# rubychen0611/image-analogies-python

Measured on AMD Instinct MI355X. Metric: B' pixels/sec (brute-force match, 5-level pyramid) + MFMA util @1/2/4/8 GPU, higher is better.
Workload: dtype f16 rotated split (R16 MFMA screen: 3 principal components as f16 pairs, 52 as f16, f32 accumulate) + f64 (rotation, exact rescore, pyramids); 1 GPU; c4: A/A' 2048x2048 x B 1024x1024, 5-level, DB sharded, brute force; levels_cap=5, jobs_per_gpu=1, streams_per_gpu=1, jobs_per_launch=1, parallelism=single

## Files before the change

### image-analogies-python_amd/csrc/ia_screen16r.hip

```cpp
#include "ia_internal.h"
#include "ia_rot16.h"
#include "../../include/ia_diag.h"

#include <float.h>
#include <type_traits>

namespace ia {
namespace {

typedef float floatx16 __attribute__((ext_vector_type(16)));
constexpr int STAGE_TILES = 4;
constexpr int STAGE_H8 = STAGE_TILES * R16_TILE_H8;
constexpr int MAX_G = 11;
constexpr int SPC_MAX = 16;
#ifndef IA_R16_RING
#define IA_R16_RING 2
#endif
#ifndef IA_R16_OCC
#define IA_R16_OCC 4
#endif
constexpr int R16_RING = IA_R16_RING;
#ifndef IA_R16_NTMIN
#define IA_R16_NTMIN 0
#endif
#ifndef IA_R16_PIN
#define IA_R16_PIN 1
#endif
#ifndef IA_R16_SPC
#define IA_R16_SPC 2
#endif
constexpr int SPC_STAGE = IA_R16_SPC;
#ifndef IA_RK_TILES
#define IA_RK_TILES 4
#endif
#ifndef IA_RK_RING
#define IA_RK_RING 2
#endif
#ifndef IA_RK_SPC
#define IA_RK_SPC 8
#endif
#ifndef IA_RK_OCC
#define IA_RK_OCC 4
#endif
constexpr int RK_TILES = IA_RK_TILES, RK_RING = IA_RK_RING, RK_SPC = IA_RK_SPC;
static_assert(RK_TILES == 4 || RK_TILES == 8, "a compact stage is one or two 128-row stages of the stage map");
static_assert(RK_RING >= 2 && R16_RING >= 2 && RK_SPC >= 1 && RK_SPC <= 16, "stage ring, staged minima");

__host__ __device__ constexpr int bal_t0(int G, int W) { return (G * W) / 4; }
__host__ __device__ constexpr int bal_ns(int G, int W) { return (G * W + G - 1) / 4 - (G * W) / 4 + 1; }
__host__ __device__ constexpr bool bal_on(int G, int W, int k, int u) {
    return 4 * (bal_t0(G, W) + k) + u >= G * W && 4 * (bal_t0(G, W) + k) + u < G * W + G;
}
template <int G, int W>
__host__ __device__ constexpr int ch_count() {
    int n = 0;
    for (int u = 0; u < STAGE_TILES; ++u)
        for (int k = 0; k < bal_ns(G, W); ++k) n += bal_on(G, W, k, u) ? 1 : 0;
    return n;
}
template <int G, int W>
__host__ __device__ constexpr int ch_u(int c) {
    for (int u = 0; u < STAGE_TILES; ++u)
        for (int k = 0; k < bal_ns(G, W); ++k)
            if (bal_on(G, W, k, u) && c-- == 0) return u;
    return -1;
}
template <int G, int W>
__host__ __device__ constexpr int ch_k(int c) {
    for (int u = 0; u < STAGE_TILES; ++u)
        for (int k = 0; k < bal_ns(G, W); ++k)
            if (bal_on(G, W, k, u) && c-- == 0) return k;
    return -1;
}
template <int G, int W>
__host__ __device__ constexpr int ch_uo(int c) {
    int o = 0;
    for (int i = 1; i <= c; ++i) o += ch_u<G, W>(i) != ch_u<G, W>(i - 1) ? 1 : 0;
    return o;
}
template <int G, int W>
__host__ __device__ constexpr int ch_next(int c) {
    for (int i = c + 1; i < ch_count<G, W>(); ++i)
        if (ch_u<G, W>(i) != ch_u<G, W>(c)) return i;
    return -1;
}
template <int G, int W>
__host__ __device__ constexpr bool ch_first(int c) { return c == 0 || ch_u<G, W>(c) != ch_u<G, W>(c - 1); }
#ifndef IA_R16_PF
#define IA_R16_PF 1
#endif
template <int G, int W>
__host__ __device__ constexpr bool ch_reads_next(int c) {
    return IA_R16_PF ? (ch_first<G, W>(c) && ch_next<G, W>(c) >= 0)
                     : (c + 1 < ch_count<G, W>() && ch_u<G, W>(c + 1) != ch_u<G, W>(c));
}
template <int K, int N, typename F>
__device__ __forceinline__ void sfor(F &&f) {
    if constexpr (K < N) {
        f(std::integral_constant<int, K>{});
        sfor<K + 1, N>(f);
    }
}
__device__ __forceinline__ int fkey(float x) {
    const int b = __float_as_int(x);
    return b >= 0 ? b : b ^ 0x7fffffff;
}
__device__ __forceinline__ float fkey_inv(int b) { return __int_as_float(b >= 0 ? b : b ^ 0x7fffffff); }
__device__ __forceinline__ void fold_min(const floatx16 &x, float &mn) {
    const float t0 = fminf(fminf(x[0], x[1]), x[2]), t1 = fminf(fminf(x[3], x[4]), x[5]);
    const float t2 = fminf(fminf(x[6], x[7]), x[8]), t3 = fminf(fminf(x[9], x[10]), x[11]);
    const float t4 = fminf(fminf(x[12], x[13]), x[14]);
    const float u0 = fminf(fminf(t0, t1), t2), u1 = fminf(fminf(t3, t4), x[15]);
    mn = fminf(fminf(mn, u0), u1);
}

#ifndef IA_R16_LAG
#define IA_R16_LAG 2
#endif
constexpr int R16_NACC = IA_R16_LAG + 1;

template <int G, int W, int NS>
__device__ __forceinline__ void r16_stage(const half8 *sb, const half8 (&bq)[NS][R16_MFMA], float (&mn)[NS],
                                          int lane) {
    constexpr int NC = ch_count<G, W>();
    const floatx16 zero = {};
    half8 a[2][R16_MFMA];
    floatx16 acc[R16_NACC];
    {
        const half8 *p = sb + ch_u<G, W>(0) * R16_TILE_H8 + lane;
#pragma unroll
        for (int m = 0; m < R16_MFMA; ++m) a[0][m] = p[m * 64];
    }
    sfor<0, NC>([&](auto cc) {
        constexpr int c = decltype(cc)::value;
        constexpr int k = ch_k<G, W>(c), ab = ch_uo<G, W>(c) & 1, cb = c % R16_NACC;
        constexpr int cf = c - IA_R16_LAG, fb = (c + 1) % R16_NACC;
        if constexpr (ch_reads_next<G, W>(c)) {
            const half8 *p = sb + ch_u<G, W>(ch_next<G, W>(c)) * R16_TILE_H8 + lane;
#pragma unroll
            for (int m = 0; m < R16_MFMA; ++m) a[ab ^ 1][m] = p[m * 64];
        }
        acc[cb] = __builtin_amdgcn_mfma_f32_32x32x16_f16(a[ab][0], bq[k][0], zero, 0, 0, 0);
        if constexpr (cf >= 0) fold_min(acc[fb], mn[ch_k<G, W>(cf)]);
#pragma unroll
        for (int m = 1; m < R16_MFMA; ++m)
            acc[cb] = __builtin_amdgcn_mfma_f32_32x32x16_f16(a[ab][m], bq[k][m], acc[cb], 0, 0, 0);
        if constexpr (IA_R16_PIN) {
            if constexpr (ch_reads_next<G, W>(c))
                __builtin_amdgcn_sched_group_barrier(0x100, R16_MFMA, 0);
            __builtin_amdgcn_sched_group_barrier(0x008, 1, 0);
            if constexpr (cf >= 0) {
                sfor<0, R16_MFMA - 1>([&](auto) {
                    __builtin_amdgcn_sched_group_barrier(0x002, 2, 0);
                    __builtin_amdgcn_sched_group_barrier(0x008, 1, 0);
                });
            } else {
                __builtin_amdgcn_sched_group_barrier(0x008, R16_MFMA - 1, 0);
            }
            __builtin_amdgcn_sched_barrier(0);
        }
    });
    sfor<(NC > IA_R16_LAG ? NC - IA_R16_LAG : 0), NC>([&](auto cc) {
        constexpr int c = decltype(cc)::value;
        fold_min(acc[c % R16_NACC], mn[ch_k<G, W>(c)]);
    });
}

typedef float floatx4 __attribute__((ext_vector_type(4)));
template <int G, int W>
__host__ __device__ constexpr int c16_lo() { return 4 * G * W; }
template <int G, int W>
__host__ __device__ constexpr int c16_t0() { return c16_lo<G, W>() / 8; }
template <int G, int W>
__host__ __device__ constexpr int c16_ns() { return (c16_lo<G, W>() + 4 * G - 1) / 8 - c16_t0<G, W>() + 1; }
template <int G, int W>
__host__ __device__ constexpr bool c16_on(int k, int v) {
    return 8 * (c16_t0<G, W>() + k) + v >= c16_lo<G, W>() && 8 * (c16_t0<G, W>() + k) + v < c16_lo<G, W>() + 4 * G;
}
template <int G, int W>
__host__ __device__ constexpr int c16_count() { return 4 * G; }
template <int G, int W>
__host__ __device__ constexpr int c16_v(int c) {
    for (int v = 0; v < 8; ++v)
        for (int k = 0; k < c16_ns<G, W>(); ++k)
            if (c16_on<G, W>(k, v) && c-- == 0) return v;
    return -1;
}
template <int G, int W>
__host__ __device__ constexpr int c16_k(int c) {
    for (int v = 0; v < 8; ++v)
        for (int k = 0; k < c16_ns<G, W>(); ++k)
            if (c16_on<G, W>(k, v) && c-- == 0) return k;
    return -1;
}
template <int G, int W>
__host__ __device__ constexpr int c16_vo(int c) {
    int o = 0;
    for (int i = 1; i <= c; ++i) o += c16_v<G, W>(i) != c16_v<G, W>(i - 1) ? 1 : 0;
    return o;
}
template <int G, int W>
__host__ __device__ constexpr int c16_next(int c) {
    for (int i = c + 1; i < c16_count<G, W>(); ++i)
        if (c16_v<G, W>(i) != c16_v<G, W>(c)) return i;
    return -1;
}
template <int G, int W>
__host__ __device__ constexpr bool c16_first(int c) { return c == 0 || c16_v<G, W>(c) != c16_v<G, W>(c - 1); }
__device__ __forceinline__ int s16_aoff(int v, int n, int lane) {
    const int q = lane >> 4, r = lane & 15;
    return (v >> 1) * R16_TILE_H8 + ((2 * n + (q >> 1)) * 64 + (q & 1) * 32 + 16 * (v & 1) + r);
}
constexpr int S16_LAG = 3;
constexpr int S16_NACC = S16_LAG + 1;

template <int G, int W, int NS>
__device__ __forceinline__ void r16_stage_s16(const half8 *sb, const half8 (&bq)[NS][2], float (&mn)[NS], int lane) {
    constexpr int NC = c16_count<G, W>();
    const floatx4 zero = {};
    half8 a[2][2];
    floatx4 acc[S16_NACC];
    a[0][0] = sb[s16_aoff(c16_v<G, W>(0), 0, lane)];
    a[0][1] = sb[s16_aoff(c16_v<G, W>(0), 1, lane)];
    sfor<0, NC>([&](auto cc) {
        constexpr int c = decltype(cc)::value;
        constexpr int k = c16_k<G, W>(c), ab = c16_vo<G, W>(c) & 1, cb = c % S16_NACC;
        constexpr int cf = c - S16_LAG, fb = (c + 1) % S16_NACC;
        constexpr bool rd = c16_first<G, W>(c) && c16_next<G, W>(c) >= 0;
        if constexpr (rd) {
            constexpr int vn = c16_v<G, W>(c16_next<G, W>(c));
            a[ab ^ 1][0] = sb[s16_aoff(vn, 0, lane)];
            a[ab ^ 1][1] = sb[s16_aoff(vn, 1, lane)];
        }
        acc[cb] = __builtin_amdgcn_mfma_f32_16x16x32_f16(a[ab][0], bq[k][0], zero, 0, 0, 0);
        if constexpr (cf >= 0) mn[c16_k<G, W>(cf)] = fminf(mn[c16_k<G, W>(cf)], fminf(acc[fb][0], acc[fb][1]));
        acc[cb] = __builtin_amdgcn_mfma_f32_16x16x32_f16(a[ab][1], bq[k][1], acc[cb], 0, 0, 0);
        if constexpr (cf >= 0) mn[c16_k<G, W>(cf)] = fminf(mn[c16_k<G, W>(cf)], fminf(acc[fb][2], acc[fb][3]));
        if constexpr (IA_R16_PIN) {
            if constexpr (rd) __builtin_amdgcn_sched_group_barrier(0x100, 2, 0);
            __builtin_amdgcn_sched_group_barrier(0x008, 1, 0);
            if constexpr (cf >= 0) __builtin_amdgcn_sched_group_barrier(0x002, 1, 0);
            __builtin_amdgcn_sched_group_barrier(0x008, 1, 0);
            if constexpr (cf >= 0) __builtin_amdgcn_sched_group_barrier(0x002, 1, 0);
            __builtin_amdgcn_sched_barrier(0);
        }
    });
    sfor<(NC > S16_LAG ? NC - S16_LAG : 0), NC>([&](auto cc) {
        constexpr int c = decltype(cc)::value;
        const floatx4 &x = acc[c % S16_NACC];
        mn[c16_k<G, W>(c)] = fminf(fminf(mn[c16_k<G, W>(c)], fminf(x[0], x[1])), fminf(x[2], x[3]));
    });
}

__device__ __forceinline__ int s16k_aoff(int v, int lane) {
    return (v >> 1) * RK_TILE_H8 + (lane >> 4) * 32 + 16 * (v & 1) + (lane & 15);
}
template <int G, int W, int NS>
__device__ __forceinline__ void r16_stage_s16k(const half8 *sb, const half8 (&bq)[NS][1], float (&mn)[NS], int lane) {
    constexpr int NC = c16_count<G, W>();
    const floatx4 zero = {};
    half8 a[2];
    floatx4 acc[S16_NACC];
    a[0] = sb[s16k_aoff(c16_v<G, W>(0), lane)];
    sfor<0, NC>([&](auto cc) {
        constexpr int c = decltype(cc)::value;
        constexpr int k = c16_k<G, W>(c), ab = c16_vo<G, W>(c) & 1, cb = c % S16_NACC;
        constexpr int cf = c - S16_LAG, fb = (c + 1) % S16_NACC;
        constexpr bool rd = c16_first<G, W>(c) && c16_next<G, W>(c) >= 0;
        if constexpr (rd) a[ab ^ 1] = sb[s16k_aoff(c16_v<G, W>(c16_next<G, W>(c)), lane)];
        acc[cb] = __builtin_amdgcn_mfma_f32_16x16x32_f16(a[ab], bq[k][0], zero, 0, 0, 0);
        if constexpr (cf >= 0) {
            constexpr int kf = c16_k<G, W>(cf);
            mn[kf] = fminf(fminf(mn[kf], fminf(acc[fb][0], acc[fb][1])), fminf(acc[fb][2], acc[fb][3]));
        }
        if constexpr (IA_R16_PIN) {
            if constexpr (rd) __builtin_amdgcn_sched_group_barrier(0x100, 1, 0);
            __builtin_amdgcn_sched_group_barrier(0x008, 1, 0);
            if constexpr (cf >= 0) __builtin_amdgcn_sched_group_barrier(0x002, 2, 0);
            __builtin_amdgcn_sched_barrier(0);
        }
    });
    sfor<(NC > S16_LAG ? NC - S16_LAG : 0), NC>([&](auto cc) {
        constexpr int c = decltype(cc)::value;
        const floatx4 &x = acc[c % S16_NACC];
        mn[c16_k<G, W>(c)] = fminf(fminf(mn[c16_k<G, W>(c)], fminf(x[0], x[1])), fminf(x[2], x[3]));
    });
}

__device__ __forceinline__ void lds_min_i32(int *p, int v) {
    typedef __attribute__((address_space(3))) int lds_int;
    const unsigned a = (unsigned)(unsigned long)(lds_int *)p;
    asm volatile("ds_min_i32 %0, %1" :: "v"(a), "v"(v) : "memory");
}

template <int G, int W, int NS>
__device__ __forceinline__ void r16_close(int s, int tps, int *smin, float (&mn)[NS], int lane) {
    constexpr int T0 = bal_t0(G, W);
    const int done = (s + 1) * STAGE_TILES;
    if (done % tps == 0) {
        int *sm = smin + ((done / tps - 1) % SPC_STAGE) * (G * 32);
        const int j = lane & 31, h = lane >> 5;
#pragma unroll
        for (int k = 0; k < NS; ++k) {
            const float m = fminf(mn[k], __shfl_xor(mn[k], 32));
            if (h == 0) lds_min_i32(&sm[(T0 + k) * 32 + j], fkey(m));
            mn[k] = FLT_MAX;
        }
    }
}
template <int G, int W, int NS, int TILES = STAGE_TILES, int SPC = SPC_STAGE>
__device__ __forceinline__ void r16_close_s16(int s, int tps, int *smin, float (&mn)[NS], int lane) {
    constexpr int T0 = c16_t0<G, W>();
    const int done = (s + 1) * TILES;
    if (done % tps == 0) {
        int *sm = smin + ((done / tps - 1) % SPC) * (G * 32);
#pragma unroll
        for (int k = 0; k < NS; ++k) {
            float m = fminf(mn[k], __shfl_xor(mn[k], 16));
            m = fminf(m, __shfl_xor(m, 32));
            if (lane < 16) lds_min_i32(&sm[(T0 + k) * 16 + lane], fkey(m));
            mn[k] = FLT_MAX;
        }
    }
}

__device__ __forceinline__ void stage_barrier() {
    asm volatile("s_waitcnt lgkmcnt(0)" ::: "memory");
    __builtin_amdgcn_s_barrier();
    asm volatile("" ::: "memory");
}


template <int NP, int MAXA>
__device__ __forceinline__ void wait_stages(int ahead) {
    if constexpr (MAXA == 0) {
        asm volatile("s_waitcnt vmcnt(0)" ::: "memory");
    } else {
        static_assert(NP * MAXA < 64, "vmcnt is a 6-bit count");
        if (ahead >= MAXA) asm volatile("s_waitcnt vmcnt(%0)" :: "n"(NP * MAXA) : "memory");
        else wait_stages<NP, MAXA - 1>(ahead);
    }
}

template <int G, int W, bool CMP = false, int TILES = STAGE_TILES>
__device__ __forceinline__ void r16_body(const half8 *__restrict__ db16, half8 *sbuf, int *smin,
                                         const StageMap &sm, long chunk, int s0, int nstage, int tps,
                                         const half8 *__restrict__ q16, float *__restrict__ segmin,
                                         long seg0, long nseg, int q0, int M) {
    static_assert(!CMP || RK_BUILT, "the compact form needs the 16x16x32 shape at P = 3");
    static_assert(TILES % STAGE_TILES == 0 && (CMP || TILES == STAGE_TILES), "stage geometry");
    constexpr int RING = CMP ? RK_RING : R16_RING, SPC = CMP ? RK_SPC : SPC_STAGE;
    constexpr int MS = TILES / STAGE_TILES;
    constexpr int NS = R16_S16 ? c16_ns<G, W>() : bal_ns(G, W);
    constexpr int T0 = bal_t0(G, W);
    constexpr int TH8 = CMP ? RK_TILE_H8 : R16_TILE_H8, MH8 = STAGE_TILES * TH8, SH8 = MS * MH8;
    constexpr int NPM = MH8 / 256, NP = MS * NPM;
    const int tid = threadIdx.x;
    const int lane = tid & 63;
    half8 bq[NS][CMP ? 1 : R16_S16 ? 2 : R16_MFMA];
    if constexpr (CMP) {
#pragma unroll
        for (int k = 0; k < NS; ++k)
            bq[k][0] = q16[(long)((c16_t0<G, W>() + k) * 16 + (lane & 15)) * Q16_ROW + RK_Q_F16 / 8 + (lane >> 4)];
    } else if constexpr (R16_S16) {
        const int q = lane >> 4, c = lane & 15;
#pragma unroll
        for (int k = 0; k < NS; ++k) {
            const half8 *p = q16 + (long)((c16_t0<G, W>() + k) * 16 + c) * Q16_ROW + (q & 1) * R16_MFMA + (q >> 1);
            bq[k][0] = p[0];
            bq[k][1] = p[2];
        }
    } else {
        const int j = lane & 31, h = lane >> 5;
#pragma unroll
        for (int k = 0; k < NS; ++k) {
            const half8 *p = q16 + (long)((T0 + k) * 32 + j) * Q16_ROW + h * R16_MFMA;
#pragma unroll
            for (int m = 0; m < R16_MFMA; ++m) bq[k][m] = p[m];
        }
    }
    auto issue = [&](int s) {
        if constexpr (MS == 1) {
            const half8 *src = db16 + (stage_lrow(sm, chunk, s0 + s) >> 5) * TH8 + W * 64 + lane;
            half8 *dst = sbuf + (s % RING) * SH8 + W * 64;
#pragma unroll
            for (int k = 0; k < NP; ++k)
                __builtin_amdgcn_global_load_lds((const void *)(src + k * 256), (void *)(dst + k * 256), 16, 0, 2);
        } else {
#pragma unroll
            for (int h = 0; h < MS; ++h) {
                const half8 *src = db16 + (stage_lrow(sm, chunk, s0 + s * MS + h) >> 5) * TH8 + W * 64 + lane;
                half8 *dst = sbuf + (s % RING) * SH8 + h * MH8 + W * 64;
#pragma unroll
                for (int k = 0; k < NPM; ++k)
                    __builtin_amdgcn_global_load_lds((const void *)(src + k * 256), (void *)(dst + k * 256), 16, 0,
                                                     2);
            }
        }
    };
    float mn[NS];
#pragma unroll
    for (int k = 0; k < NS; ++k) mn[k] = FLT_MAX;
    const int spc = nstage * TILES / tps;
#pragma unroll
    for (int s = 0; s < RING - 1; ++s)
        if (s < nstage) issue(s);
    if constexpr (CMP) wait_stages<NP, RING - 2>(nstage - 1);
    else if (nstage > 1) asm volatile("s_waitcnt vmcnt(%0)" :: "n"(NP * (RING - 2)) : "memory");
    else asm volatile("s_waitcnt vmcnt(0)" ::: "memory");
    stage_barrier();
    for (int s = 0; s < nstage; ++s) {
        const bool more = s + RING - 1 < nstage;
        if (more) issue(s + RING - 1);
        if constexpr (CMP) {
#pragma nounroll
            for (int h = 0; h < MS; ++h)
                r16_stage_s16k<G, W, NS>(sbuf + (s % RING) * SH8 + h * MH8, bq, mn, lane);
            r16_close_s16<G, W, NS, TILES, SPC>(s, tps, smin, mn, lane);
        } else if constexpr (R16_S16) {
            r16_stage_s16<G, W, NS>(sbuf + (s % RING) * SH8, bq, mn, lane);
            r16_close_s16<G, W, NS>(s, tps, smin, mn, lane);
        } else {
            r16_stage<G, W, NS>(sbuf + (s % RING) * SH8, bq, mn, lane);
            r16_close<G, W, NS>(s, tps, smin, mn, lane);
        }
        const int done = (s + 1) * TILES;
        if (done % tps == 0) {
            const int sg = done / tps - 1;
            if (sg % SPC == SPC - 1 || sg == spc - 1) {
                stage_barrier();
                const int base = sg - sg % SPC, n = sg - base + 1;
                for (int i = tid; i < G * 32 * n; i += 256) {
                    const int ql = i / n, k = i - ql * n;
                    int *e = &smin[k * (G * 32) + ql];
                    if (q0 + ql < M) {
                        float *dst = segmin + ((long)(q0 + ql) * nseg + seg0 + base + k);
                        if constexpr (IA_R16_NTMIN) __builtin_nontemporal_store(fkey_inv(*e), dst);
                        else *dst = fkey_inv(*e);
                    }
                    *e = 0x7fffffff;
                }
            }
        }
        if constexpr (CMP) wait_stages<NP, RING - 2>(nstage - 2 - s);
        else if (more) asm volatile("s_waitcnt vmcnt(%0)" :: "n"(NP * (RING - 2)) : "memory");
        else asm volatile("s_waitcnt vmcnt(0)" ::: "memory");
        stage_barrier();
    }
}

template <int G>
__global__ __launch_bounds__(256, IA_R16_OCC) void k_screen16r(const half8 *__restrict__ db16, int nchunks, int ch,
                                                      int seg_rows, StageMap sm,
                                                      const half8 *__restrict__ q16, int M, int groups,
                                                      float *__restrict__ segmin, long nseg,
                                                      const XJob *jobs, int parity, int split) {
    __shared__ half8 sbuf[R16_RING * STAGE_H8];
    __shared__ int smin[SPC_STAGE * G * 32];
    if (jobs) {
        const XJob &J = jobs[blockIdx.y];
        db16 = reinterpret_cast<const half8 *>(J.dbr.get());
        q16 = reinterpret_cast<const half8 *>(J.q16[parity].get());
        segmin = J.segmin;
    }
    const int b = blockIdx.x;
    const int slot = b >> 3;
    const int part = (slot / groups) * 8 + (b & 7);
    const int group = slot - (slot / groups) * groups;
    if (part >= nchunks * split) return;
    const int lsp = __builtin_ctz((unsigned)split);
    const int chunk = part >> lsp, half = part & (split - 1);
    const int spc = ch / seg_rows;
    for (int i = threadIdx.x; i < SPC_STAGE * G * 32; i += 256) smin[i] = 0x7fffffff;
    const int nstage = (ch / (STAGE_TILES * 32)) >> lsp;
    const int tps = seg_rows >> 5;
    const half8 *qg = q16 + (long)group * G * 32 * Q16_ROW;
    const long seg0 = (long)chunk * spc + (long)half * (spc >> lsp);
    const int q0 = group * G * 32;
    const int s0 = half * nstage;
    const int wv = __builtin_amdgcn_readfirstlane(threadIdx.x >> 6);
    if (wv == 0) r16_body<G, 0>(db16, sbuf, smin, sm, chunk, s0, nstage, tps, qg, segmin, seg0, nseg, q0, M);
    else if (wv == 1) r16_body<G, 1>(db16, sbuf, smin, sm, chunk, s0, nstage, tps, qg, segmin, seg0, nseg, q0, M);
    else if (wv == 2) r16_body<G, 2>(db16, sbuf, smin, sm, chunk, s0, nstage, tps, qg, segmin, seg0, nseg, q0, M);
    else r16_body<G, 3>(db16, sbuf, smin, sm, chunk, s0, nstage, tps, qg, segmin, seg0, nseg, q0, M);
}

__host__ __device__ inline void sq_split(int nT, int qg, int &first, int &count) {
    const int ng = (nT + MAX_G - 1) / MAX_G, base = nT / ng, rem = nT - base * ng;
    first = qg * base + (qg < rem ? qg : rem);
    count = base + (qg < rem ? 1 : 0);
}

template <int G, int W>
__device__ __forceinline__ void r16_body_s(const half8 *__restrict__ db16, half8 *sbuf, int *smin,
                                           const StageMap &sm, long chunk, int s0, int nstage, int tps,
                                           const half8 *const *qt, float *const *sp, const int *lim,
                                           long seg0, long nseg) {
    constexpr int NS = R16_S16 ? c16_ns<G, W>() : bal_ns(G, W);
    constexpr int T0 = bal_t0(G, W);
    constexpr int TH8 = R16_TILE_H8, SH8 = STAGE_TILES * TH8, NP = SH8 / 256;
    const int tid = threadIdx.x;
    const int lane = tid & 63;
    half8 bq[NS][R16_S16 ? 2 : R16_MFMA];
    if constexpr (R16_S16) {
        const int q = lane >> 4, c = lane & 15;
#pragma unroll
        for (int k = 0; k < NS; ++k) {
            constexpr int B0 = c16_t0<G, W>();
            const half8 *p = qt[(B0 + k) >> 1] + (long)(((B0 + k) & 1) * 16 + c) * Q16_ROW + (q & 1) * R16_MFMA + (q >> 1);
            bq[k][0] = p[0];
            bq[k][1] = p[2];
        }
    } else {
        const int j = lane & 31, h = lane >> 5;
#pragma unroll
        for (int k = 0; k < NS; ++k) {
            const half8 *p = qt[T0 + k] + (long)j * Q16_ROW + h * R16_MFMA;
#pragma unroll
            for (int m = 0; m < R16_MFMA; ++m) bq[k][m] = p[m];
        }
    }
    auto issue = [&](int s) {
        const half8 *src = db16 + (stage_lrow(sm, chunk, s0 + s) >> 5) * TH8 + W * 64 + lane;
        half8 *dst = sbuf + (s % R16_RING) * SH8 + W * 64;
#pragma unroll
        for (int k = 0; k < NP; ++k)
            __builtin_amdgcn_global_load_lds((const void *)(src + k * 256), (void *)(dst + k * 256), 16, 0, 2);
    };
    float mn[NS];
#pragma unroll
    for (int k = 0; k < NS; ++k) mn[k] = FLT_MAX;
    const int spc = nstage * STAGE_TILES / tps;
#pragma unroll
    for (int s = 0; s < R16_RING - 1; ++s)
        if (s < nstage) issue(s);
    if (nstage > 1) asm volatile("s_waitcnt vmcnt(%0)" :: "n"(NP * (R16_RING - 2)) : "memory");
    else asm volatile("s_waitcnt vmcnt(0)" ::: "memory");
    stage_barrier();
    for (int s = 0; s < nstage; ++s) {
        const bool more = s + R16_RING - 1 < nstage;
        if (more) issue(s + R16_RING - 1);
        if constexpr (R16_S16) {
            r16_stage_s16<G, W, NS>(sbuf + (s % R16_RING) * SH8, bq, mn, lane);
            r16_close_s16<G, W, NS>(s, tps, smin, mn, lane);
        } else {
            r16_stage<G, W, NS>(sbuf + (s % R16_RING) * SH8, bq, mn, lane);
            r16_close<G, W, NS>(s, tps, smin, mn, lane);
        }
        const int done = (s + 1) * STAGE_TILES;
        if (done % tps == 0) {
            const int sg = done / tps - 1;
            if (sg % SPC_STAGE == SPC_STAGE - 1 || sg == spc - 1) {
                stage_barrier();
                const int base = sg - sg % SPC_STAGE, n = sg - base + 1;
                for (int i = tid; i < G * 32 * n; i += 256) {
                    const int ql = i / n, k = i - ql * n;
                    int *e = &smin[k * (G * 32) + ql];
                    const int tl = ql >> 5, l = ql & 31;
                    if (l < lim[tl]) {
                        float *dst = sp[tl] + ((long)l * nseg + seg0 + base + k);
                        if constexpr (IA_R16_NTMIN) __builtin_nontemporal_store(fkey_inv(*e), dst);
                        else *dst = fkey_inv(*e);
                    }
                    *e = 0x7fffffff;
                }
            }
        }
        if (more) asm volatile("s_waitcnt vmcnt(%0)" :: "n"(NP * (R16_RING - 2)) : "memory");
        else asm volatile("s_waitcnt vmcnt(0)" ::: "memory");
        stage_barrier();
    }
}

template <int G>
__global__ __launch_bounds__(256, IA_R16_OCC) void k_screen16rs(const XJob *__restrict__ jobs,
                                                       const int *__restrict__ gtab, int nchunks, int ch,
                                                       int seg_rows, StageMap sm, int M, int nqg, long nseg,
                                                       int parity, int split) {
    __shared__ half8 sbuf[R16_RING * STAGE_H8];
    __shared__ int smin[SPC_STAGE * G * 32];
    __shared__ const half8 *qt[G];
    __shared__ float *sp[G];
    __shared__ int lim[G];
    const int b = blockIdx.x;
    const int slot = b >> 3;
    const int part = (slot / nqg) * 8 + (b & 7);
    if (part >= nchunks * split) return;
    const int T = (M + 31) >> 5, ngroups = gtab[0];
    int qg = slot - (slot / nqg) * nqg, g = 0, pos = 0, n = gtab[1];
    while (g + 1 < ngroups) {
        const int here = (n * T + MAX_G - 1) / MAX_G;
        if (qg < here) break;
        qg -= here;
        pos += n;
        n = gtab[1 + ++g];
    }
    int first, count;
    sq_split(n * T, qg, first, count);
    count = count < G ? count : G;
    if (first + count > n * T) first = count = 0;
    const int *order = gtab + 1 + IA_BATCH_MAX + pos;
    if (threadIdx.x < G) {
        const int i = threadIdx.x, ti = first + (i < count ? i : 0);
        const int jp = ti / T, tj = ti - jp * T;
        const XJob &J = jobs[order[jp]];
        qt[i] = reinterpret_cast<const half8 *>(J.q16[parity].get()) + (long)tj * 32 * Q16_ROW;
        sp[i] = J.segmin.get() + (long)tj * 32 * nseg;
        lim[i] = i < count ? (M - 32 * tj < 32 ? M - 32 * tj : 32) : 0;
    }
    const half8 *db16 = reinterpret_cast<const half8 *>(jobs[order[0]].dbr.get());
    const int lsp = __builtin_ctz((unsigned)split);
    const int chunk = part >> lsp, half = part & (split - 1);
    const int spc = ch / seg_rows;
    for (int i = threadIdx.x; i < SPC_STAGE * G * 32; i += 256) smin[i] = 0x7fffffff;
    const int nstage = (ch / (STAGE_TILES * 32)) >> lsp;
    const int tps = seg_rows >> 5;
    const long seg0 = (long)chunk * spc + (long)half * (spc >> lsp);
    const int s0 = half * nstage;
    __syncthreads();
    const int wv = __builtin_amdgcn_readfirstlane(threadIdx.x >> 6);
    if (wv == 0) r16_body_s<G, 0>(db16, sbuf, smin, sm, chunk, s0, nstage, tps, qt, sp, lim, seg0, nseg);
    else if (wv == 1) r16_body_s<G, 1>(db16, sbuf, smin, sm, chunk, s0, nstage, tps, qt, sp, lim, seg0, nseg);
    else if (wv == 2) r16_body_s<G, 2>(db16, sbuf, smin, sm, chunk, s0, nstage, tps, qt, sp, lim, seg0, nseg);
    else r16_body_s<G, 3>(db16, sbuf, smin, sm, chunk, s0, nstage, tps, qt, sp, lim, seg0, nseg);
}

template <int G, int TILES>
__global__ __launch_bounds__(256, IA_RK_OCC) void k_screen16c(const half8 *__restrict__ dbk, int nchunks, int ch,
                                                     int seg_rows, StageMap sm,
                                                     const half8 *__restrict__ q16, int M, int groups,
                                                     float *__restrict__ segmin, long nseg, int split) {
    __shared__ half8 sbuf[RK_RING * TILES * RK_TILE_H8];
    __shared__ int smin[RK_SPC * G * 32];
    const int b = blockIdx.x;
    const int slot = b >> 3;
    const int part = (slot / groups) * 8 + (b & 7);
    const int group = slot - (slot / groups) * groups;
    if (part >= nchunks * split) return;
    const int lsp = __builtin_ctz((unsigned)split);
    const int chunk = part >> lsp, half = part & (split - 1);
    const int spc = ch / seg_rows;
    for (int i = threadIdx.x; i < RK_SPC * G * 32; i += 256) smin[i] = 0x7fffffff;
    const int nstage = (ch / (TILES * 32)) >> lsp;
    const int tps = seg_rows >> 5;
    const half8 *qg = q16 + (long)group * G * 32 * Q16_ROW;
    const long seg0 = (long)chunk * spc + (long)half * (spc >> lsp);
    const int q0 = group * G * 32;
    const int s0 = half * nstage * (TILES / STAGE_TILES);
    const int wv = __builtin_amdgcn_readfirstlane(threadIdx.x >> 6);
    if constexpr (RK_BUILT) {
        if (wv == 0) r16_body<G, 0, true, TILES>(dbk, sbuf, smin, sm, chunk, s0, nstage, tps, qg, segmin, seg0, nseg, q0, M);
        else if (wv == 1) r16_body<G, 1, true, TILES>(dbk, sbuf, smin, sm, chunk, s0, nstage, tps, qg, segmin, seg0, nseg, q0, M);
        else if (wv == 2) r16_body<G, 2, true, TILES>(dbk, sbuf, smin, sm, chunk, s0, nstage, tps, qg, segmin, seg0, nseg, q0, M);
        else r16_body<G, 3, true, TILES>(dbk, sbuf, smin, sm, chunk, s0, nstage, tps, qg, segmin, seg0, nseg, q0, M);
    }
}

#ifndef IA_R16W_RING
#define IA_R16W_RING 3
#endif
constexpr int W_RING = IA_R16W_RING;
constexpr int W_WAVES = 8;
#ifndef IA_R16W_SPB
#define IA_R16W_SPB 16
#endif
constexpr int W_SPB_MAX = IA_R16W_SPB;
constexpr int W_LAG = 2;

__device__ __forceinline__ void w_fold(const floatx4 &x, const floatx4 &y, float &mn) {
    mn = fminf(fminf(mn, fminf(x[0], x[1])), fminf(fminf(x[2], x[3]), fminf(fminf(y[0], y[1]), fminf(y[2], y[3]))));
}

template <int NQB>
__device__ __forceinline__ void w_tile(const half8 (&a)[4], const half8 *qs, float (&mn)[NQB], int lane) {
    const floatx4 zero = {};
    half8 bq[2][2];
    floatx4 acc[W_LAG + 1][2];
    bq[0][0] = qs[lane];
    bq[0][1] = qs[64 + lane];
    sfor<0, NQB>([&](auto kk) {
        constexpr int k = decltype(kk)::value, cb = k % (W_LAG + 1), b = k & 1;
        if constexpr (k + 1 < NQB) {
            bq[b ^ 1][0] = qs[((k + 1) * 2) * 64 + lane];
            bq[b ^ 1][1] = qs[((k + 1) * 2 + 1) * 64 + lane];
        }
        acc[cb][0] = __builtin_amdgcn_mfma_f32_16x16x32_f16(a[0], bq[b][0], zero, 0, 0, 0);
        acc[cb][1] = __builtin_amdgcn_mfma_f32_16x16x32_f16(a[2], bq[b][0], zero, 0, 0, 0);
        acc[cb][0] = __builtin_amdgcn_mfma_f32_16x16x32_f16(a[1], bq[b][1], acc[cb][0], 0, 0, 0);
        acc[cb][1] = __builtin_amdgcn_mfma_f32_16x16x32_f16(a[3], bq[b][1], acc[cb][1], 0, 0, 0);
        if constexpr (k >= W_LAG) {
            constexpr int f = (k - W_LAG) % (W_LAG + 1);
            w_fold(acc[f][0], acc[f][1], mn[k - W_LAG]);
        }
    });
    sfor<(NQB > W_LAG ? NQB - W_LAG : 0), NQB>([&](auto kk) {
        constexpr int k = decltype(kk)::value;
        w_fold(acc[k % (W_LAG + 1)][0], acc[k % (W_LAG + 1)][1], mn[k]);
    });
}

template <int G>
__global__ __launch_bounds__(512, 4) void k_screen16w(const half8 *__restrict__ db16, int nsb, int spb, int tps,
                                                      int seg_rows, StageMap sm, const half8 *__restrict__ q16,
                                                      int M, int groups, float *__restrict__ segmin, long nseg,
                                                      const XJob *jobs, int parity) {
    constexpr int NQB = 2 * G;
    __shared__ half8 qs[NQB * 2 * 64];
    __shared__ int smin[W_SPB_MAX * NQB * 16];
    if (jobs) {
        const XJob &J = jobs[blockIdx.y];
        db16 = reinterpret_cast<const half8 *>(J.dbr.get());
        q16 = reinterpret_cast<const half8 *>(J.q16[parity].get());
        segmin = J.segmin;
    }
    const int b = blockIdx.x;
    const int slot = b >> 3;
    const int sbk = (slot / groups) * 8 + (b & 7);
    const int group = slot - (slot / groups) * groups;
    if (sbk >= nsb) return;
    const int tid = threadIdx.x, lane = tid & 63;
    const int wv = __builtin_amdgcn_readfirstlane(tid >> 6);
    const half8 *qg = q16 + (long)group * G * 32 * Q16_ROW;
    for (int i = tid; i < NQB * 128; i += 512) {
        const int k = i >> 7, n = (i >> 6) & 1, l = i & 63, lq = l >> 4;
        qs[i] = qg[(long)(k * 16 + (l & 15)) * Q16_ROW + (lq & 1) * R16_MFMA + (lq >> 1) + 2 * n];
    }
    for (int i = tid; i < spb * NQB * 16; i += 512) smin[i] = 0x7fffffff;
    __syncthreads();
    const long seg0 = (long)sbk * spb;
    const int tpw = spb * tps / W_WAVES;
    const int jw = wv * tpw;
    const int lts = __builtin_ctz((unsigned)tps);
    const int q = lane >> 4, r = lane & 15;
    const int o0 = (q >> 1) * 64 + (q & 1) * 32 + r;
    auto tile = [&](int j) -> const half8 * {
        j = j < tpw ? j : tpw - 1;
        const int jj = jw + j;
        const long lrow = seg_lrow(sm, seg0 + (jj >> lts), seg_rows, (long)(jj & (tps - 1)) * 32);
        return db16 + (lrow >> 5) * R16_TILE_H8 + o0;
    };
    half8 a[W_RING][4];
    auto issue = [&](half8 (&d)[4], int j) {
        const half8 *t = tile(j);
        d[0] = __builtin_nontemporal_load(t);
        d[1] = __builtin_nontemporal_load(t + 128);
        d[2] = __builtin_nontemporal_load(t + 16);
        d[3] = __builtin_nontemporal_load(t + 144);
    };
    float mn[NQB];
#pragma unroll
    for (int k = 0; k < NQB; ++k) mn[k] = FLT_MAX;
    sfor<0, W_RING - 1>([&](auto ss) { issue(a[decltype(ss)::value], decltype(ss)::value); });
    for (int j0 = 0; j0 < tpw; j0 += W_RING) {
        sfor<0, W_RING>([&](auto ss) {
            constexpr int s = decltype(ss)::value;
            const int j = j0 + s;
            issue(a[(s + W_RING - 1) % W_RING], j + W_RING - 1);
            if (j < tpw) {
                w_tile<NQB>(a[s], qs, mn, lane);
                const int jj = jw + j;
                if (((jj + 1) & (tps - 1)) == 0 || j + 1 == tpw) {
                    int *sm0 = smin + (jj >> lts) * (NQB * 16);
#pragma unroll
                    for (int k = 0; k < NQB; ++k) {
                        float m = fminf(mn[k], __shfl_xor(mn[k], 16));
                        m = fminf(m, __shfl_xor(m, 32));
                        if (lane < 16) lds_min_i32(&sm0[k * 16 + lane], fkey(m));
                        mn[k] = FLT_MAX;
                    }
                }
            }
        });
    }
    stage_barrier();
    const int q0 = group * G * 32;
    for (int i = tid; i < NQB * 16 * spb; i += 512) {
        const int ql = i / spb, k = i - ql * spb;
        if (q0 + ql < M) segmin[(long)(q0 + ql) * nseg + seg0 + k] = fkey_inv(smin[k * (NQB * 16) + ql]);
    }
}

constexpr int COV_ROWS = 128, COV_PAIRS = 55 * 56 / 2, COV_BLOCKS = 256;
__global__ __launch_bounds__(256) void k_db_cov(DbSrc src, long row0, long nrows, long step, long nsamp,
                                                const double *__restrict__ center, double *__restrict__ part) {
    __shared__ double X[COV_ROWS][IA_DP];
    double acc[(COV_PAIRS + 255) / 256];
#pragma unroll
    for (int i = 0; i < (COV_PAIRS + 255) / 256; ++i) acc[i] = 0.0;
    for (long base = (long)blockIdx.x * COV_ROWS; base < nsamp; base += (long)gridDim.x * COV_ROWS) {
        __syncthreads();
        if (threadIdx.x < COV_ROWS) {
            const long i = base + threadIdx.x;
            double *x = X[threadIdx.x];
            if (i < nsamp) {
                ImgPair a, ap; int r, c;
                src.locate(row0 + i * step, a, ap, r, c);
                emit_feature(a, ap, r, c, [&](int k, double v) { x[k] = v - center[k]; });
            } else {
                for (int k = 0; k < IA_D; ++k) x[k] = 0.0;
            }
        }
        __syncthreads();
#pragma unroll
        for (int i = 0; i < (COV_PAIRS + 255) / 256; ++i) {
            const int p = threadIdx.x + 256 * i;
            if (p < COV_PAIRS) {
                int a = 0, rem = p;
                while (rem >= 55 - a) { rem -= 55 - a; ++a; }
                const int bb = a + rem;
                double s = 0.0;
                for (int r = 0; r < COV_ROWS; ++r) s += X[r][a] * X[r][bb];
                acc[i] += s;
            }
        }
    }
#pragma unroll
    for (int i = 0; i < (COV_PAIRS + 255) / 256; ++i) {
        const int p = threadIdx.x + 256 * i;
        if (p < COV_PAIRS) part[(long)blockIdx.x * COV_PAIRS + p] = acc[i];
    }
}
__global__ __launch_bounds__(256) void k_db_cov_reduce(const double *__restrict__ part, int nb, double *__restrict__ cov) {
    for (int p = threadIdx.x; p < COV_PAIRS; p += 256) {
        double s = 0.0;
        for (int b = 0; b < nb; ++b) s += part[(long)b * COV_PAIRS + p];
        int a = 0, rem = p;
        while (rem >= 55 - a) { rem -= 55 - a; ++a; }
        const int bb = a + rem;
        cov[a * R16_LD + bb] = s;
        cov[bb * R16_LD + a] = s;
    }
}

template <typename F>
__device__ __forceinline__ void r16_rotate_row(const float *R, const double (&d)[IA_D], F &&f) {
#pragma unroll
    for (int jb = 0; jb < R16_LD; jb += 4) {
        double k0 = 0.0, k1 = 0.0, k2 = 0.0, k3 = 0.0;
#pragma unroll
        for (int k = 0; k < IA_D; ++k) {
            const float4 v = *reinterpret_cast<const float4 *>(&R[k * R16_LD + jb]);
            k0 = fma((double)v.x, d[k], k0);
            k1 = fma((double)v.y, d[k], k1);
            k2 = fma((double)v.z, d[k], k2);
            k3 = fma((double)v.w, d[k], k3);
        }
        const double kk[4] = {k0, k1, k2, k3};
#pragma unroll
        for (int e = 0; e < 4; ++e)
            if (jb + e < IA_D) f(jb + e, kk[e]);
    }
}
// ... 242 lines not shown
    const int ch = db_chunk_rows(nrows);
    const long nchunks = db_nchunks(nrows);
    const int seg_rows = db_seg_rows(nrows);
    const long nseg = db_nsegs(nrows);
    IA_ARG(M > 0 && ch % (STAGE_TILES * 32) == 0 && seg_rows % (STAGE_TILES * 32) == 0 &&
               ch / seg_rows <= SPC_MAX,
           "launch_screen16rs: bad chunking");
    IA_ARG(sm.sc == ch / 128, "launch_screen16rs: stage map of another chunking");
    IA_ARG(jobs && gtab && gcount && ngroups >= 1 && ngroups <= IA_BATCH_MAX, "launch_screen16rs: bad batch");
    int G = 0;
    const int nqg = shared_qgroups(gcount, ngroups, M, &G);
    static const long cus = [] {
        int dev = 0, n = 0;
        if (hipGetDevice(&dev) != hipSuccess || hipDeviceGetAttribute(&n, hipDeviceAttributeMultiprocessorCount, dev) != hipSuccess || n <= 0)
            n = 256;
        return (long)n;
    }();
    const int spc = ch / seg_rows;
    int split = 1;
    while (2 * split <= spc && nchunks * 2 * split * nqg <= cus * IA_R16_OCC) split *= 2;
    const long nb = ((nchunks * split + 7) / 8) * 8 * nqg;
    IA_ARG(nb < (1L << 31), "screen grid too large");
#define IA_R16S_CASE(GG)                                                                            \
    case GG:                                                                                        \
        k_screen16rs<GG><<<(unsigned)nb, 256, 0, st>>>(jobs, gtab, (int)nchunks, ch, seg_rows, sm, M, \
                                                       nqg, nseg, parity, split);                   \
        break;
    switch (G) {
        IA_R16S_CASE(1)
        IA_R16S_CASE(2)
        IA_R16S_CASE(3)
        IA_R16S_CASE(4)
        IA_R16S_CASE(5)
        IA_R16S_CASE(6)
        IA_R16S_CASE(7)
        IA_R16S_CASE(8)
        IA_R16S_CASE(9)
        IA_R16S_CASE(10)
        IA_R16S_CASE(11)
        default: set_error("launch_screen16rs: bad query split"); return IA_E_ARG;
    }
#undef IA_R16S_CASE
    IA_LAUNCH_CHECK("k_screen16rs");
    return IA_OK;
}

int launch_query_rows_r16(const double *q64, int M, const double *center, const float *rot,
                          const float *amax, double *nq, double *nsk, _Float16 *q16, hipStream_t st,
                          bool compact = false) {
    k_query_rows_r16<<<M, 64, 0, st>>>(q64, center, rot, amax, nq, nsk, q16, compact);
    IA_LAUNCH_CHECK("k_query_rows_r16");
    return IA_OK;
}

int launch_db_amax(const IaSrcLevel *src, const DbSrc &d, const double *center, float *amax,
                   double *part, hipStream_t st);
int screen16i_attributes(hipFuncAttributes *at);
int screen_resources_r16(hipFuncAttributes *at) {
    IA_HIP(hipFuncGetAttributes(at, reinterpret_cast<const void *>(&k_screen16r<11>)));
    return IA_OK;
}

}

using namespace ia;

extern "C" {

int ia_db_rot_applies(const IaSrcLevel *src, long row0, long nrows) {
    if (!src || nrows <= 0 || row0 < 0 || !src_nA_ok(*src)) return 0;
    return row0 + nrows <= (long)src->nAp * src->Ah * src->Aw ? 1 : 0;
}

int ia_screen_resources(int which, int *lds, int *vgprs) {
    IA_ARG(lds && vgprs && (which == 0 || which == 1), "ia_screen_resources: bad args");
    hipFuncAttributes at{};
    const int rc = which == 0 ? screen_resources_r16(&at) : screen16i_attributes(&at);
    if (rc) return rc;
    *lds = (int)at.sharedSizeBytes;
    *vgprs = at.numRegs;
    return IA_OK;
}

int ia_diag_set_r16_form(int form) {
    const int prev = r16_form();
    if (form == 0 || form == 1) g_r16_form.store(form);
    return prev;
}

int ia_diag_shared_screen_groups(const int *jobs_per_group, int G, int M, int *out) {
    IA_ARG(jobs_per_group && G >= 1 && G <= IA_BATCH_MAX && M > 0, "ia_diag_shared_screen_groups: bad args");
    int K = 0;
    for (int g = 0; g < G; ++g) {
        IA_ARG(jobs_per_group[g] >= 1, "ia_diag_shared_screen_groups: an empty DB group");
        K += jobs_per_group[g];
    }
    IA_ARG(K <= IA_BATCH_MAX, "ia_diag_shared_screen_groups: more than 128 jobs");
    const int T = (M + 31) / 32;
    int nqg = 0;
    for (int g = 0; g < G; ++g) {
        const int nT = jobs_per_group[g] * T, ng = (nT + MAX_G - 1) / MAX_G;
        for (int qg = 0; qg < ng; ++qg, ++nqg) {
            if (!out) continue;
            int *o = out + (size_t)nqg * IA_SHARED_QG_INTS;
            int first, count;
            sq_split(nT, qg, first, count);
            o[0] = g; o[1] = first; o[2] = count;
            for (int i = 0; i < MAX_G; ++i) {
                o[3 + 2 * i] = i < count ? (first + i) / T : -1;
                o[4 + 2 * i] = i < count ? (first + i) % T : -1;
            }
        }
    }
    return nqg;
}

int ia_db_rot_components(void) { return R16_P; }
int ia_db_rotk_span(int *kept, int *axes, int cap) {
    if (kept) *kept = RK_BUILT ? RK_C : 0;
    if (!RK_BUILT) return 0;
    for (int i = 0; axes && i < RK_NAXES && i < cap; ++i) axes[i] = RK_AXES[i];
    return RK_NAXES;
}
int ia_db_rot_slots(void) { return R16_SLOTS; }
double ia_db_rot_eps_a2(void) { return R16_EPS_A2; }

size_t ia_db_rot_bytes(long nrows) { return nrows > 0 ? r16_askc_off(nrows) + img_align((size_t)db_nsegs(nrows)) : 0; }

size_t ia_db_cov_bytes(void) { return (size_t)(R16_LD * R16_LD + COV_BLOCKS * COV_PAIRS) * sizeof(double); }

int ia_db_cov(const IaSrcLevel *src, long row0, long nrows, const double *center, double *cov, void *stream) {
    IA_ARG(src && center && cov && nrows > 0 && row0 >= 0, "ia_db_cov: bad args");
    IA_SRC_NA(*src, "ia_db_cov");
    IA_ARG(row0 + nrows <= (long)src->nAp * src->Ah * src->Aw, "ia_db_cov: rows out of range");
    hipStream_t st = S(stream);
    const DbSrc d = make_dbsrc(*src);
    const long step = (nrows / 65536) | 1;
    const long nsamp = (nrows + step - 1) / step;
    double *part = cov + R16_LD * R16_LD;
    const int nb = (int)std::min<long>(COV_BLOCKS, (nsamp + COV_ROWS - 1) / COV_ROWS);
    IA_HIP(hipMemsetAsync(cov, 0, (size_t)R16_LD * R16_LD * sizeof(double), st));
    k_db_cov<<<nb, 256, 0, st>>>(d, row0, nrows, step, nsamp, center, part);
    IA_LAUNCH_CHECK("k_db_cov");
    k_db_cov_reduce<<<1, 256, 0, st>>>(part, nb, cov);
    IA_LAUNCH_CHECK("k_db_cov_reduce");
    return IA_OK;
}

int ia_db_build_rot(const IaSrcLevel *src, long row0, long nrows, const double *center, const float *rot,
                    float *amax, void *dbr, void *stream) {
    IA_ARG(src && center && rot && amax && dbr && nrows > 0 && row0 >= 0, "ia_db_build_rot: bad args");
    IA_SRC_NA(*src, "ia_db_build_rot");
    IA_ARG(row0 + nrows <= (long)src->nAp * src->Ah * src->Aw, "ia_db_build_rot: rows out of range");
    IA_ARG(row0 + nrows < (1L << 31), "ia_db_build_rot: rows past 2^31");
    hipStream_t st = S(stream);
    {
        const int rc = rot_check_orthonormal(rot, IA_D, R16_LD, st, "ia_db_build_rot");
        if (rc) return rc;
    }
    const DbSrc d = make_dbsrc(*src);
    const long npad = db_rows_padded(nrows);
    IA_ARG(npad * (long)R16_ROW_B >= 1024L * 8 * 8, "ia_db_build_rot: too few rows for the bound's partials");
    const int rc = launch_db_amax(src, d, center, amax, reinterpret_cast<double *>(dbr), st);
    if (rc) return rc;
    const StageMap sm = db_stage_map(row0, nrows, src->Aw, src->Ah);
    const long nseg = db_nsegs(nrows);
// ... 86 lines not shown
```

Measured before the change: 2.178 million B' pixels/s.

## Chain min folds, close blocks via permlane swaps, vectorize segmin flush, add stamps

Min folds over MFMA accumulators become a serial chain of fminf calls, used in the compact path and the W kernel. Block close-out in the compact and W paths packs four query blocks into one lane-swap reduction using permlane16/32 swaps, replacing shuffles and cutting the number of LDS atomics. In the compact path, segment minima are flushed with 16-byte vector stores when the alignment allows it. Optional timestamp instrumentation is also added but compiled out by default. The main s16 path explicitly keeps the old fold and close forms.

```diff
diff --git a/image-analogies-python_amd/csrc/ia_screen16r.hip b/image-analogies-python_amd/csrc/ia_screen16r.hip
--- a/image-analogies-python_amd/csrc/ia_screen16r.hip
+++ b/image-analogies-python_amd/csrc/ia_screen16r.hip
@@ -30,6 +30,9 @@
 #define IA_R16_SPC 2
 #endif
 constexpr int SPC_STAGE = IA_R16_SPC;
+#ifndef IA_R16_FLUSH
+#define IA_R16_FLUSH 1
+#endif
 #ifndef IA_RK_TILES
 #define IA_RK_TILES 4
 #endif
@@ -167,6 +170,18 @@
 }
 
 typedef float floatx4 __attribute__((ext_vector_type(4)));
+#ifndef IA_R16_FOLD
+#define IA_R16_FOLD 1
+#endif
+template <bool CH = IA_R16_FOLD>
+__device__ __forceinline__ float fold2(float mn, float a, float b) {
+    return CH ? fminf(fminf(mn, a), b) : fminf(mn, fminf(a, b));
+}
+template <bool CH = IA_R16_FOLD>
+__device__ __forceinline__ float fold4(float mn, const floatx4 &x) {
+    return CH ? fold2<true>(fold2<true>(mn, x[0], x[1]), x[2], x[3])
+              : fminf(fminf(mn, fminf(x[0], x[1])), fminf(x[2], x[3]));
+}
 template <int G, int W>
 __host__ __device__ constexpr int c16_lo() { return 4 * G * W; }
 template <int G, int W>
@@ -214,7 +229,7 @@
 constexpr int S16_LAG = 3;
 constexpr int S16_NACC = S16_LAG + 1;
 
-template <int G, int W, int NS>
+template <int G, int W, int NS, bool CH = IA_R16_FOLD>
 __device__ __forceinline__ void r16_stage_s16(const half8 *sb, const half8 (&bq)[NS][2], float (&mn)[NS], int lane) {
     constexpr int NC = c16_count<G, W>();
     const floatx4 zero = {};
@@ -233,9 +248,9 @@
             a[ab ^ 1][1] = sb[s16_aoff(vn, 1, lane)];
         }
         acc[cb] = __builtin_amdgcn_mfma_f32_16x16x32_f16(a[ab][0], bq[k][0], zero, 0, 0, 0);
-        if constexpr (cf >= 0) mn[c16_k<G, W>(cf)] = fminf(mn[c16_k<G, W>(cf)], fminf(acc[fb][0], acc[fb][1]));
+        if constexpr (cf >= 0) mn[c16_k<G, W>(cf)] = fold2<CH>(mn[c16_k<G, W>(cf)], acc[fb][0], acc[fb][1]);
         acc[cb] = __builtin_amdgcn_mfma_f32_16x16x32_f16(a[ab][1], bq[k][1], acc[cb], 0, 0, 0);
-        if constexpr (cf >= 0) mn[c16_k<G, W>(cf)] = fminf(mn[c16_k<G, W>(cf)], fminf(acc[fb][2], acc[fb][3]));
+        if constexpr (cf >= 0) mn[c16_k<G, W>(cf)] = fold2<CH>(mn[c16_k<G, W>(cf)], acc[fb][2], acc[fb][3]);
         if constexpr (IA_R16_PIN) {
             if constexpr (rd) __builtin_amdgcn_sched_group_barrier(0x100, 2, 0);
             __builtin_amdgcn_sched_group_barrier(0x008, 1, 0);
@@ -247,8 +262,7 @@
     });
     sfor<(NC > S16_LAG ? NC - S16_LAG : 0), NC>([&](auto cc) {
         constexpr int c = decltype(cc)::value;
-        const floatx4 &x = acc[c % S16_NACC];
-        mn[c16_k<G, W>(c)] = fminf(fminf(mn[c16_k<G, W>(c)], fminf(x[0], x[1])), fminf(x[2], x[3]));
+        mn[c16_k<G, W>(c)] = fold4<CH>(mn[c16_k<G, W>(c)], acc[c % S16_NACC]);
     });
 }
 
@@ -271,7 +285,7 @@
         acc[cb] = __builtin_amdgcn_mfma_f32_16x16x32_f16(a[ab], bq[k][0], zero, 0, 0, 0);
         if constexpr (cf >= 0) {
             constexpr int kf = c16_k<G, W>(cf);
-            mn[kf] = fminf(fminf(mn[kf], fminf(acc[fb][0], acc[fb][1])), fminf(acc[fb][2], acc[fb][3]));
+            mn[kf] = fold4(mn[kf], acc[fb]);
         }
         if constexpr (IA_R16_PIN) {
             if constexpr (rd) __builtin_amdgcn_sched_group_barrier(0x100, 1, 0);
@@ -282,8 +296,7 @@
     });
     sfor<(NC > S16_LAG ? NC - S16_LAG : 0), NC>([&](auto cc) {
         constexpr int c = decltype(cc)::value;
-        const floatx4 &x = acc[c % S16_NACC];
-        mn[c16_k<G, W>(c)] = fminf(fminf(mn[c16_k<G, W>(c)], fminf(x[0], x[1])), fminf(x[2], x[3]));
+        mn[c16_k<G, W>(c)] = fold4(mn[c16_k<G, W>(c)], acc[c % S16_NACC]);
     });
 }
 
@@ -308,20 +321,45 @@
         }
     }
 }
-template <int G, int W, int NS, int TILES = STAGE_TILES, int SPC = SPC_STAGE>
+#ifndef IA_R16_CLOSE
+#define IA_R16_CLOSE 1
+#endif
+__device__ __forceinline__ float swap_min16(float a, float b) {
+    const auto r = __builtin_amdgcn_permlane16_swap(__float_as_uint(a), __float_as_uint(b), false, false);
+    return fminf(__uint_as_float(r[0]), __uint_as_float(r[1]));
+}
+__device__ __forceinline__ float swap_min32(float a, float b) {
+    const auto r = __builtin_amdgcn_permlane32_swap(__float_as_uint(a), __float_as_uint(b), false, false);
+    return fminf(__uint_as_float(r[0]), __uint_as_float(r[1]));
+}
+template <int NS, bool SW = IA_R16_CLOSE>
+__device__ __forceinline__ void close_blocks_s16(int *sm, float (&mn)[NS], int lane) {
+    if constexpr (SW) {
+        sfor<0, (NS + 3) / 4>([&](auto ii) {
+            constexpr int k0 = 4 * decltype(ii)::value, n = NS - k0 < 4 ? NS - k0 : 4;
+            constexpr int k1 = k0 + (n > 1 ? 1 : 0), k2 = k0 + (n > 2 ? 2 : n - 1), k3 = k0 + n - 1;
+            const float p = swap_min16(mn[k0], mn[k1]);
+            const float q = n > 2 ? swap_min16(mn[k2], mn[k3]) : p;
+            const int m = fkey(swap_min32(p, q));
+            if (n == 4 || lane < 16 * n) lds_min_i32(&sm[k0 * 16 + lane], m);
+        });
+#pragma unroll
+        for (int k = 0; k < NS; ++k) mn[k] = FLT_MAX;
+    } else {
+#pragma unroll
+        for (int k = 0; k < NS; ++k) {
+            float m = fminf(mn[k], __shfl_xor(mn[k], 16));
+            m = fminf(m, __shfl_xor(m, 32));
+            if (lane < 16) lds_min_i32(&sm[k * 16 + lane], fkey(m));
+            mn[k] = FLT_MAX;
+        }
+    }
+}
+template <int G, int W, int NS, int TILES = STAGE_TILES, int SPC = SPC_STAGE, bool SW = IA_R16_CLOSE>
 __device__ __forceinline__ void r16_close_s16(int s, int tps, int *smin, float (&mn)[NS], int lane) {
     constexpr int T0 = c16_t0<G, W>();
     const int done = (s + 1) * TILES;
-    if (done % tps == 0) {
-        int *sm = smin + ((done / tps - 1) % SPC) * (G * 32);
-#pragma unroll
-        for (int k = 0; k < NS; ++k) {
-            float m = fminf(mn[k], __shfl_xor(mn[k], 16));
-            m = fminf(m, __shfl_xor(m, 32));
-            if (lane < 16) lds_min_i32(&sm[(T0 + k) * 16 + lane], fkey(m));
-            mn[k] = FLT_MAX;
-        }
-    }
+    if (done % tps == 0) close_blocks_s16<NS, SW>(smin + ((done / tps - 1) % SPC) * (G * 32) + T0 * 16, mn, lane);
 }
 
 __device__ __forceinline__ void stage_barrier() {
@@ -341,6 +379,14 @@
         else wait_stages<NP, MAXA - 1>(ahead);
     }
 }
+
+#ifndef IA_R16_STAMPS
+#define IA_R16_STAMPS 0
+#endif
+#if IA_R16_STAMPS
+constexpr int ST_BLOCKS = 8, ST_STAGES = 64, ST_POINTS = 5;
+__device__ unsigned long long g_r16_stamps[ST_BLOCKS][ST_STAGES][ST_POINTS];
+#endif
 
 template <int G, int W, bool CMP = false, int TILES = STAGE_TILES>
 __device__ __forceinline__ void r16_body(const half8 *__restrict__ db16, half8 *sbuf, int *smin,
@@ -402,6 +448,22 @@
 #pragma unroll
     for (int k = 0; k < NS; ++k) mn[k] = FLT_MAX;
     const int spc = nstage * TILES / tps;
+#if IA_R16_STAMPS
+    const int st_stride = gridDim.x >= ST_BLOCKS ? gridDim.x / ST_BLOCKS : 1;
+    const int st_slot = CMP && W == 0 && blockIdx.x % st_stride == 0 && blockIdx.x / st_stride < ST_BLOCKS
+                            ? (int)(blockIdx.x / st_stride) : -1;
+    __shared__ unsigned long long st_lds[ST_STAGES * ST_POINTS];
+    auto stamp = [&](int s, int i) {
+        if (st_slot >= 0 && s < ST_STAGES) {
+            typedef __attribute__((address_space(3))) unsigned long long lds_u64;
+            const unsigned long long t = __builtin_amdgcn_s_memtime();
+            const unsigned a = (unsigned)(unsigned long)(lds_u64 *)&st_lds[s * ST_POINTS + i];
+            asm volatile("ds_write_b64 %0, %1" :: "v"(a), "v"(t) : "memory");
+        }
+    };
+#else
+    auto stamp = [](int, int) {};
+#endif
 #pragma unroll
     for (int s = 0; s < RING - 1; ++s)
         if (s < nstage) issue(s);
@@ -411,15 +473,17 @@
     stage_barrier();
     for (int s = 0; s < nstage; ++s) {
         const bool more = s + RING - 1 < nstage;
+        stamp(s, 0);
         if (more) issue(s + RING - 1);
         if constexpr (CMP) {
 #pragma nounroll
             for (int h = 0; h < MS; ++h)
                 r16_stage_s16k<G, W, NS>(sbuf + (s % RING) * SH8 + h * MH8, bq, mn, lane);
+            stamp(s, 1);
             r16_close_s16<G, W, NS, TILES, SPC>(s, tps, smin, mn, lane);
         } else if constexpr (R16_S16) {
-            r16_stage_s16<G, W, NS>(sbuf + (s % RING) * SH8, bq, mn, lane);
-            r16_close_s16<G, W, NS>(s, tps, smin, mn, lane);
+            r16_stage_s16<G, W, NS, false>(sbuf + (s % RING) * SH8, bq, mn, lane);
+            r16_close_s16<G, W, NS, STAGE_TILES, SPC_STAGE, false>(s, tps, smin, mn, lane);
         } else {
             r16_stage<G, W, NS>(sbuf + (s % RING) * SH8, bq, mn, lane);
             r16_close<G, W, NS>(s, tps, smin, mn, lane);
@@ -430,23 +494,65 @@
             if (sg % SPC == SPC - 1 || sg == spc - 1) {
                 stage_barrier();
                 const int base = sg - sg % SPC, n = sg - base + 1;
-                for (int i = tid; i < G * 32 * n; i += 256) {
-                    const int ql = i / n, k = i - ql * n;
-                    int *e = &smin[k * (G * 32) + ql];
-                    if (q0 + ql < M) {
-                        float *dst = segmin + ((long)(q0 + ql) * nseg + seg0 + base + k);
-                        if constexpr (IA_R16_NTMIN) __builtin_nontemporal_store(fkey_inv(*e), dst);
-                        else *dst = fkey_inv(*e);
+                float *out = segmin + (seg0 + base);
+                if constexpr (!CMP) {
+                    for (int i = tid; i < G * 32 * n; i += 256) {
+                        const int ql = i / n, k = i - ql * n;
+                        int *e = &smin[k * (G * 32) + ql];
+                        if (q0 + ql < M) {
+                            float *dst = segmin + ((long)(q0 + ql) * nseg + seg0 + base + k);
+                            if constexpr (IA_R16_NTMIN) __builtin_nontemporal_store(fkey_inv(*e), dst);
+                            else *dst = fkey_inv(*e);
+                        }
+                        *e = 0x7fffffff;
                     }
-                    *e = 0x7fffffff;
+                } else if (IA_R16_FLUSH && SPC % 4 == 0 && n == SPC && ((nseg | (seg0 + base)) & 3) == 0 &&
+                           ((unsigned long)segmin & 15) == 0) {
+                    constexpr int PC = SPC / 4;
+                    for (int i = tid; i < G * 32 * PC; i += 256) {
+                        const int ql = ((i >> 5) / PC) * 32 + (i & 31), h = (i >> 5) % PC;
+                        int *e = &smin[4 * h * (G * 32) + ql];
+                        floatx4 v;
+#pragma unroll
+                        for (int j = 0; j < 4; ++j) {
+                            v[j] = fkey_inv(e[j * (G * 32)]);
+                            e[j * (G * 32)] = 0x7fffffff;
+                        }
+                        if (q0 + ql < M) {
+                            floatx4 *dst = reinterpret_cast<floatx4 *>(out + (long)(q0 + ql) * nseg + 4 * h);
+                            if constexpr (IA_R16_NTMIN) __builtin_nontemporal_store(v, dst);
+                            else *dst = v;
+                        }
+                    }
+                } else {
+                    for (int i = tid; i < G * 32 * n; i += 256) {
+                        const int ql = i / n, k = i - ql * n;
+                        int *e = &smin[k * (G * 32) + ql];
+                        if (q0 + ql < M) {
+                            float *dst = out + ((long)(q0 + ql) * nseg + k);
+                            if constexpr (IA_R16_NTMIN) __builtin_nontemporal_store(fkey_inv(*e), dst);
+                            else *dst = fkey_inv(*e);
+                        }
+                        *e = 0x7fffffff;
+                    }
                 }
             }
         }
+        stamp(s, 2);
         if constexpr (CMP) wait_stages<NP, RING - 2>(nstage - 2 - s);
         else if (more) asm volatile("s_waitcnt vmcnt(%0)" :: "n"(NP * (RING - 2)) : "memory");
         else asm volatile("s_waitcnt vmcnt(0)" ::: "memory");
+        stamp(s, 3);
         stage_barrier();
-    }
+        stamp(s, 4);
+    }
+#if IA_R16_STAMPS
+    if (st_slot >= 0) {
+        asm volatile("s_waitcnt lgkmcnt(0)" ::: "memory");
+        for (int i = lane; i < ST_STAGES * ST_POINTS; i += 64)
+            (&g_r16_stamps[st_slot][0][0])[i] = i / ST_POINTS < nstage ? st_lds[i] : 0ull;
+    }
+#endif
 }
 
 template <int G>
@@ -541,8 +647,8 @@
         const bool more = s + R16_RING - 1 < nstage;
         if (more) issue(s + R16_RING - 1);
         if constexpr (R16_S16) {
-            r16_stage_s16<G, W, NS>(sbuf + (s % R16_RING) * SH8, bq, mn, lane);
-            r16_close_s16<G, W, NS>(s, tps, smin, mn, lane);
+            r16_stage_s16<G, W, NS, false>(sbuf + (s % R16_RING) * SH8, bq, mn, lane);
+            r16_close_s16<G, W, NS, STAGE_TILES, SPC_STAGE, false>(s, tps, smin, mn, lane);
         } else {
             r16_stage<G, W, NS>(sbuf + (s % R16_RING) * SH8, bq, mn, lane);
             r16_close<G, W, NS>(s, tps, smin, mn, lane);
@@ -668,7 +774,8 @@
 constexpr int W_LAG = 2;
 
 __device__ __forceinline__ void w_fold(const floatx4 &x, const floatx4 &y, float &mn) {
-    mn = fminf(fminf(mn, fminf(x[0], x[1])), fminf(fminf(x[2], x[3]), fminf(fminf(y[0], y[1]), fminf(y[2], y[3]))));
+    if constexpr (IA_R16_FOLD) mn = fold4(fold4(mn, x), y);
+    else mn = fminf(fminf(mn, fminf(x[0], x[1])), fminf(fminf(x[2], x[3]), fminf(fminf(y[0], y[1]), fminf(y[2], y[3]))));
 }
 
 template <int NQB>
@@ -760,14 +867,7 @@
                 w_tile<NQB>(a[s], qs, mn, lane);
                 const int jj = jw + j;
                 if (((jj + 1) & (tps - 1)) == 0 || j + 1 == tpw) {
-                    int *sm0 = smin + (jj >> lts) * (NQB * 16);
-#pragma unroll
-                    for (int k = 0; k < NQB; ++k) {
-                        float m = fminf(mn[k], __shfl_xor(mn[k], 16));
-                        m = fminf(m, __shfl_xor(m, 32));
-                        if (lane < 16) lds_min_i32(&sm0[k * 16 + lane], fkey(m));
-                        mn[k] = FLT_MAX;
-                    }
+                    close_blocks_s16<NQB>(smin + (jj >> lts) * (NQB * 16), mn, lane);
                 }
             }
         });
@@ -1176,6 +1276,18 @@
     return IA_OK;
 }
 
+#if IA_R16_STAMPS
+int ia_lab_r16_stamps(unsigned long long *out) {
+    IA_ARG(out, "ia_lab_r16_stamps: null buffer");
+    IA_HIP(hipDeviceSynchronize());
+    IA_HIP(hipMemcpyFromSymbol(out, HIP_SYMBOL(g_r16_stamps), sizeof(g_r16_stamps)));
+    void *p = nullptr;
+    IA_HIP(hipGetSymbolAddress(&p, HIP_SYMBOL(g_r16_stamps)));
+    IA_HIP(hipMemset(p, 0, sizeof(g_r16_stamps)));
+    return IA_OK;
+}
+#endif
+
 int ia_diag_set_r16_form(int form) {
     const int prev = r16_form();
     if (form == 0 || form == 1) g_r16_form.store(form);
```

Measured after the change: 2.305 million B' pixels/s (median of 6 runs). +5.8%, better.
